# PKU-EPIC/PartManip

Hardware: AMD Instinct MI355X
Metric: PPO env-steps/sec (whole node), 4096 envs x 1024-pt clouds (higher is better)
Workload: dtype f32

## Files before the change

### partmanip_amd/csrc/pointnet_enc_screen.h

```cpp
#pragma once

typedef __bf16 ps_bf16x8 __attribute__((ext_vector_type(8)));

#define PS_LDP (PN_C2 + 8)
#define PS_CAP 128
#define PS_NW 8
#define PS_P3 (16 * 16 * 64 * 8)
#define PS_OFF_P3H 0
#define PS_OFF_P3L (2 * PS_P3)
#define PS_OFF_W3 (4 * PS_P3 + 8192)
#define PS_OFF_EPS (PS_OFF_W3 + PN_C3 * PN_C2 * 4)
#define PS_PACKED_BYTES (PS_OFF_EPS + PN_C3 * 4)
#ifndef PS_ABLATE
#define PS_ABLATE 0
#endif
#ifndef PS_SCHED_DEFAULT
#define PS_SCHED_DEFAULT 0
#endif

extern "C" size_t pm_pointnet_packed_screen_bytes(void) { return PS_PACKED_BYTES; }

__device__ __forceinline__ unsigned ps_cvt_pk(float a, float b) {
    unsigned r;
    asm("v_cvt_pk_bf16_f32 %0, %1, %2" : "=v"(r) : "v"(a), "v"(b));
    return r;
}
__device__ __forceinline__ void ps_split(float x, unsigned short& hi, unsigned short& lo) {
    const unsigned h = ps_cvt_pk(x, 0.f) & 0xffffu;
    const float xh = __uint_as_float(h << 16);
    hi = (unsigned short)h;
    lo = (unsigned short)(ps_cvt_pk(x - xh, 0.f) & 0xffffu);
}

__global__ __launch_bounds__(256) void ps_pack_kernel(const float* __restrict__ W3, const float* __restrict__ b3,
                                                       unsigned char* __restrict__ packed) {
    const int i = blockIdx.x * 256 + threadIdx.x;
    if (i >= PS_P3) return;
    unsigned short* Ph = (unsigned short*)(packed + PS_OFF_P3H);
    unsigned short* Pl = (unsigned short*)(packed + PS_OFF_P3L);
    float* Wr = (float*)(packed + PS_OFF_W3);
    const int e = i & 7, lane = (i >> 3) & 63, li = lane & 31, lq = lane >> 5, step = (i >> 9) & 15, nb = i >> 13;
    unsigned short h, l;
    ps_split(W3[(nb * 32 + li) * PN_C2 + step * 16 + lq * 8 + e], h, l);
    Ph[i] = h;
    Pl[i] = l;
    Wr[i] = W3[i];
    if (i < 4096) ((unsigned short*)(packed + 4 * PS_P3))[i] = 0;
    if (i < PN_C3) {
        double L = 0.0;
        for (int k = 0; k < PN_C2; ++k) L += fabs((double)W3[i * PN_C2 + k]);
        const double ed = (0x1p-16 + 2048.0 * 0x1p-24) * (L + fabs((double)b3[i])) * (1.0 + 0x1p-10);
        float ef = (float)ed;
        if ((double)ef < ed) ef = __uint_as_float(__float_as_uint(ef) + 1);
        ((float*)(packed + PS_OFF_EPS))[i] = ef;
    }
}

extern "C" int pm_pointnet_pack_weights_screen(const float* W3, const float* b3, void* packed, void* stream) {
    PM_REQUIRE(W3 && b3 && packed);
    if (((uintptr_t)packed & 15) != 0) return PM_EALIGN;
    hipLaunchKernelGGL(ps_pack_kernel, dim3(PS_P3 / 256), dim3(256), 0, pm_stream(stream), W3, b3, (unsigned char*)packed);
    PM_CHECK_LAUNCH();
    return PM_OK;
}

#define PS_MFMA(a, b, c) __builtin_amdgcn_mfma_f32_32x32x16_bf16((a), (b), (c), 0, 0, 0)
__device__ __forceinline__ ps_bf16x8 ps_bf(const uint4& v) { return *(const ps_bf16x8*)&v; }

__device__ __forceinline__ void ps_stream(const unsigned short* __restrict__ Ah, const unsigned short* __restrict__ Al,
                                          const uint4* __restrict__ Bh, const uint4* __restrict__ Bl, f32x16 (&acc)[2][2]) {
    uint4 bh0[2], bl0[2], bh1[2], bl1[2];
#pragma unroll
    for (int nb = 0; nb < 2; ++nb) {
        bh0[nb] = Bh[(size_t)(nb * 16) * 64];
        bl0[nb] = Bl[(size_t)(nb * 16) * 64];
    }
#define PS_STEP(S_, BHC, BLC, BHN, BLN)                                                        \
    {                                                                                          \
        uint4 ah[2], al[2];                                                                    \
        _Pragma("unroll") for (int mb = 0; mb < 2; ++mb) {                                     \
            ah[mb] = *(const uint4*)(Ah + mb * 32 * PS_LDP + (S_) * 16);                       \
            al[mb] = *(const uint4*)(Al + mb * 32 * PS_LDP + (S_) * 16);                       \
        }                                                                                      \
        _Pragma("unroll") for (int nb = 0; nb < 2; ++nb) {    \
            BHN[nb] = Bh[(size_t)(nb * 16 + (S_) + 1) * 64];                                   \
            BLN[nb] = Bl[(size_t)(nb * 16 + (S_) + 1) * 64];                                   \
        }                                                                                      \
        __builtin_amdgcn_sched_barrier(0);                                                     \
        _Pragma("unroll") for (int nb = 0; nb < 2; ++nb)                                       \
            _Pragma("unroll") for (int mb = 0; mb < 2; ++mb) {                                 \
                acc[mb][nb] = PS_MFMA(ps_bf(ah[mb]), ps_bf(BHC[nb]), acc[mb][nb]);             \
                acc[mb][nb] = PS_MFMA(ps_bf(ah[mb]), ps_bf(BLC[nb]), acc[mb][nb]);             \
                acc[mb][nb] = PS_MFMA(ps_bf(al[mb]), ps_bf(BHC[nb]), acc[mb][nb]);             \
            }                                                                                  \
        __builtin_amdgcn_sched_barrier(0);                                                     \
    }
#pragma unroll 1
    for (int s = 0; s < 16; s += 2) {
        PS_STEP(s, bh0, bl0, bh1, bl1)
        PS_STEP(s + 1, bh1, bl1, bh0, bl0)
    }
#undef PS_STEP
}

template <int SCHED>
__device__ __forceinline__ bool ps_late_wave(int wave) { return SCHED == 1 && __builtin_amdgcn_readfirstlane(wave) >= 4; }

template <int NT>
__device__ __forceinline__ void ps_copy_h2(const float* __restrict__ H, float* __restrict__ dst, int tid) {
#pragma unroll 2
    for (int i = 0; i < PN_TM * PN_C2 / 4 / NT; ++i) {
        const int q = tid + NT * i, row = q >> 6, c4 = q & 63;
        const f32x4 v = *(const f32x4*)(H + row * PN_LD2 + 4 * c4);
        *(f32x4*)(dst + row * PN_C2 + 4 * c4) = v;
    }
}

static_assert(PN_TM * PN_MAXC == PS_NW * 64, "one staged slot per thread");
__device__ __forceinline__ float ps_point_load(const float* __restrict__ xb, int tile, int C, int tid) {
    const int p = tid >> 3, d = tid & 7;
    return d < C ? xb[(tile * PN_TM + p) * C + d] : 0.f;
}
__device__ __forceinline__ void ps_point_store(float v, int sub_mean, const float (&cen)[3], int tid, float* __restrict__ Xs) {
    const int d = tid & 7;
    if (sub_mean && d < 3) v -= cen[d];
    Xs[tid] = v;
}

#ifdef PS_PROFILE
__device__ unsigned long long ps_prof[4 * 16 * PS_NW * 16];
extern "C" int pm_debug_ps_prof_read(void* dst) {
    return hipMemcpyFromSymbol(dst, HIP_SYMBOL(ps_prof), sizeof(ps_prof)) == hipSuccess ? 0 : 1;
}
#define PS_STAMP(i)                                                                                         \
    if (b < 4 && tile < 16 && lane0 == 0) ps_prof[((b * 16 + tile) * PS_NW + wave) * 16 + (i)] = __builtin_readcyclecounter()
#else
#define PS_STAMP(i)
#endif

template <int CT, int SCHED>
__global__ __launch_bounds__(PS_NW * 64, 2) void pn_fwd_screen_kernel(
    const float* __restrict__ x, long ldx, int P, int C, int sub_mean, const float* __restrict__ W1,
    const float* __restrict__ b1, const float* __restrict__ b2, const float* __restrict__ b3,
    const float* __restrict__ packed, const unsigned char* __restrict__ packed_s, int max_mean, float* __restrict__ feat,
    long ldf, int32_t* __restrict__ argmax, float* __restrict__ h2_save, unsigned long long* __restrict__ counters) {
    constexpr int NT = PS_NW * 64;
    __shared__ __attribute__((aligned(16))) float H[PN_TM * PN_LD2];
    __shared__ __attribute__((aligned(16))) unsigned short Hp[2 * PN_TM * PS_LDP];
    __shared__ __attribute__((aligned(16))) float Xs[PN_TM * PN_MAXC];
    __shared__ double red[16];
    __shared__ double cs[PN_C2];
    __shared__ int skey[PS_NW][PS_CAP];
    unsigned short* Hh = Hp;
    unsigned short* Hl = Hp + PN_TM * PS_LDP;

    const int b = blockIdx.x, tid = threadIdx.x, lane0 = tid & 63, wave = tid >> 6;
    const float* xb = x + (long)b * ldx;
    const float4* P2v = (const float4*)(packed + PN_P2_OFF);
    const float4* P3v = (const float4*)(packed + PN_P3_OFF);
    const uint4* S3h = (const uint4*)(packed_s + PS_OFF_P3H);
    const uint4* S3l = (const uint4*)(packed_s + PS_OFF_P3L);
    const float* W3r = (const float*)(packed_s + PS_OFF_W3);
    const float* epsg = (const float*)(packed_s + PS_OFF_EPS);

    float cen[3] = {0.f, 0.f, 0.f};
    if (sub_mean) cloud_centroid<NT>(xb, P, C, red, cen);

    float vmax = -INFINITY, pois = 0.f;
    int imax = 0;
    double csum = 0.0;

    const int li0 = lane0 & 31;
    const float b2r = b2[wave * 32 + li0];
    const float b3r[2] = {b3[(wave * 2 + 0) * 32 + li0], b3[(wave * 2 + 1) * 32 + li0]};
    const float epsr[2] = {epsg[(wave * 2 + 0) * 32 + li0], epsg[(wave * 2 + 1) * 32 + li0]};
    float w1r[4] = {0.f, 0.f, 0.f, 0.f}, b1r = 0.f;
    if constexpr (CT == 3 || CT == 4) layer1_row<CT>(W1, b1, w1r, b1r);

    const int ntiles = P / PN_TM;
    stage_points<PN_TM, NT>(xb, 0, C, sub_mean, cen, Xs);
    for (int tile = 0; tile < ntiles; ++tile) {
        int lane = lane0;
        asm volatile("" : "+v"(lane));
        const int li = lane & 31, lh = lane >> 5;
        PS_STAMP(0);
        __syncthreads();
        float xnext = 0.f;
        if (tile + 1 < ntiles) xnext = ps_point_load(xb, tile + 1, C, tid);
        if (!(PS_ABLATE & 1)) {
            if constexpr (CT == 3 || CT == 4) layer1_tile<CT, PN_TM, NT, true>(Xs, w1r, b1r, H);
            else layer1_tile<CT, PN_TM, NT, true>(Xs, W1, b1, C, H);
        }
        PS_STAMP(1);
        __syncthreads();
        {
            f32x16 acc2[2][1];
            zero_acc<2, 1>(acc2);
            if (PS_ABLATE & 2) {
#pragma unroll
                for (int mb = 0; mb < 2; ++mb)
#pragma unroll
                    for (int r = 0; r < 16; ++r)
                        acc2[mb][0][r] = H[(mb * 32 + (r & 3) + 8 * (r >> 2) + 4 * lh) * PN_LD1 + ((wave * 32 + li) & 127)];
            } else {
                layer2_mfma<2, 1>(H, P2v, wave, lane, acc2);
            }
            PS_STAMP(2);
            __syncthreads();
            PS_STAMP(3);
            const int col = wave * 32 + li;
            const float b2c = b2r;
            float ts = 0.f;
            const bool planes = !(PS_ABLATE & 8) || tile == 0;
            const bool odd = (lane & 1) != 0;
            unsigned* Hh2 = (unsigned*)(Hh + (odd ? PS_LDP : 0) + (col & ~1));
            unsigned* Hl2 = (unsigned*)(Hl + (odd ? PS_LDP : 0) + (col & ~1));
#pragma unroll
            for (int mb = 0; mb < 2; ++mb)
#pragma unroll
                for (int r = 0; r < 16; r += 2) {
                    const float z0 = acc2[mb][0][r] + b2c, z1 = acc2[mb][0][r + 1] + b2c;
                    f32x2 v2;
                    if (PS_ABLATE & 4) {
                        v2.x = z0;
                        v2.y = z1;
                    } else {
                        v2 = pm_tanh2(z0, z1);
                    }
                    const int row0 = mb * 32 + (r & 3) + 8 * (r >> 2) + 4 * lh;
                    H[row0 * PN_LD2 + col] = v2.x;
                    H[(row0 + 1) * PN_LD2 + col] = v2.y;
                    ts += v2.x;
                    ts += v2.y;
                    const float own = odd ? v2.y : v2.x, send = odd ? v2.x : v2.y;
                    const float recv = __int_as_float(__builtin_amdgcn_update_dpp(0, __float_as_int(send), 0xB1, 0xf, 0xf, false));
                    const float a = odd ? recv : own, c = odd ? own : recv;
                    unsigned h2w, l2w;
                    if (PS_ABLATE & 4) {
                        h2w = (__float_as_uint(a) >> 16) | (__float_as_uint(c) & 0xffff0000u);
                        l2w = 0;
                    } else {
                        h2w = ps_cvt_pk(a, c);
                        l2w = ps_cvt_pk(a - __uint_as_float(h2w << 16), c - __uint_as_float(h2w & 0xffff0000u));
                    }
                    if (planes) {
                        Hh2[row0 * (PS_LDP / 2)] = h2w;
                        Hl2[row0 * (PS_LDP / 2)] = l2w;
                    }
                }
            ts += __shfl_xor(ts, 32, 64);
            csum += (double)ts;
            if (tile + 1 < ntiles) ps_point_store(xnext, sub_mean, cen, tid, Xs);
        }
        PS_STAMP(4);
        __syncthreads();
        PS_STAMP(5);

        const bool copy = h2_save && !(PS_ABLATE & 128), late = ps_late_wave<SCHED>(wave);
        float* h2dst = copy ? h2_save + ((long)b * P + (long)tile * PN_TM) * PN_C2 : nullptr;
        if (copy && late) ps_copy_h2<NT>(H, h2dst, tid);

        f32x16 acc[2][2];
#pragma unroll
        for (int nb = 0; nb < 2; ++nb) {
            const float b3c = b3r[nb];
#pragma unroll
            for (int r = 0; r < 16; ++r) acc[0][nb][r] = acc[1][nb][r] = b3c;
        }
        if (PS_ABLATE & 16) {
#pragma unroll
            for (int nb = 0; nb < 2; ++nb)
#pragma unroll
                for (int mb = 0; mb < 2; ++mb)
#pragma unroll
                    for (int r = 0; r < 16; ++r)
                        acc[mb][nb][r] += H[(mb * 32 + (r & 3) + 8 * (r >> 2) + 4 * lh) * PN_LD2 + ((wave * 64 + nb * 32 + li) & 255)];
        } else {
            ps_stream(Hh + li * PS_LDP + lh * 8, Hl + li * PS_LDP + lh * 8, S3h + (size_t)(wave * 2 * 16) * 64 + lane,
                      S3l + (size_t)(wave * 2 * 16) * 64 + lane, acc);
        }
        PS_STAMP(6);

        unsigned msk[2];
        float tmax[2];
#if (PS_ABLATE & 32) && defined(__HIP_DEVICE_COMPILE__)
#pragma unroll
        for (int nb = 0; nb < 2; ++nb) {
#pragma unroll
            for (int mb = 0; mb < 2; ++mb) asm volatile("" ::"v"(acc[mb][nb]));
            msk[nb] = 0;
            tmax[nb] = 0.f;
        }
#else
#pragma unroll
        for (int nb = 0; nb < 2; ++nb) {
            float m = -INFINITY;
#pragma unroll
            for (int mb = 0; mb < 2; ++mb)
#pragma unroll
                for (int r = 0; r < 16; ++r) m = fmaxf(m, acc[mb][nb][r]);
            m = fmaxf(m, __shfl_xor(m, 32, 64));
            const float e = epsr[nb];
            const float vm = __shfl(vmax, nb * 32 + li, 64);
            const float thr = m - 2.f * e;
            unsigned k = 0;
#pragma unroll
            for (int mb = 0; mb < 2; ++mb)
#pragma unroll
                for (int r = 0; r < 16; ++r) {
                    const float z = acc[mb][nb][r];
                    const bool s = !(z < thr) && !(z + e <= vm);
                    k |= (s ? 1u : 0u) << (mb * 16 + r);
                }
            msk[nb] = k;
            tmax[nb] = m;
        }
#endif
        const int n = __popc(msk[0]) + __popc(msk[1]);
        int incl = n;
#pragma unroll
        for (int o = 1; o < 64; o <<= 1) {
            const int t = __shfl_up(incl, o, 64);
            if (lane >= o) incl += t;
        }
        const int total = __builtin_amdgcn_readlane(incl, 63);
        PS_STAMP(7);

        if (PS_ABLATE & 64) {
            vmax = fmaxf(vmax, lh ? tmax[1] : tmax[0]);
            if (counters && lane == 0) atomicAdd(counters + 0, (unsigned long long)total);
        } else if (total <= PS_CAP) {
            int off = incl - n;
#pragma unroll
            for (int nb = 0; nb < 2; ++nb) {
                unsigned m = msk[nb];
                while (m) {
                    const int bit = __ffs(m) - 1;
                    m &= m - 1;
                    const int row = (bit >> 4) * 32 + (bit & 3) + 8 * ((bit & 15) >> 2) + 4 * lh;
                    skey[wave][off++] = (row << 6) | (nb * 32 + li);
                }
            }
            __builtin_amdgcn_wave_barrier();
            const int j = lane & 7, g = lane >> 3;
            for (int e0 = 0; e0 < total; e0 += 8) {
                const int e = e0 + g;
                const int key = (e < total) ? skey[wave][e] : 0;
                const int row = key >> 6, cl = key & 63;
                const float* hp = H + row * PN_LD2 + 4 * j;
                const float* wp = W3r + (size_t)(wave * 64 + cl) * PN_C2 + 4 * j;
                float s = 0.f;
#pragma unroll
                for (int i = 0; i < 8; ++i) {
                    const float4 w = *(const float4*)(wp + 32 * i);
                    const float4 h = *(const float4*)(hp + 32 * i);
                    s = fmaf(w.x, h.x, s);
                    s = fmaf(w.y, h.y, s);
                    s = fmaf(w.z, h.z, s);
                    s = fmaf(w.w, h.w, s);
                }
                s += __shfl_xor(s, 4, 64);
                s += __shfl_xor(s, 2, 64);
                s += __shfl_xor(s, 1, 64);
                s += b3[wave * 64 + cl];
#pragma unroll
                for (int gg = 0; gg < 8; ++gg)
                    if (e0 + gg < total) {
                        const int kk = __builtin_amdgcn_readlane(key, gg * 8);
                        const float v = __int_as_float(__builtin_amdgcn_readlane(__float_as_int(s), gg * 8));
                        if ((kk & 63) == lane) {
                            const int p = tile * PN_TM + (kk >> 6);
                            if (!(fabsf(v) < INFINITY)) pois += v;
                            if (v > vmax || (v == vmax && p < imax)) {
                                vmax = v;
                                imax = p;
                            }
                        }
                    }
            }
            if (counters) {
                const unsigned long long h0 = __ballot(msk[0] != 0), h1 = __ballot(msk[1] != 0);
                if (lane == 0) {
                    atomicAdd(counters + 0, (unsigned long long)total);
                    atomicAdd(counters + 2, (unsigned long long)(__popc((unsigned)(h0 | (h0 >> 32))) + __popc((unsigned)(h1 | (h1 >> 32)))));
                }
            }
        } else {
#pragma unroll
            for (int nb = 0; nb < 2; ++nb) {
                const float b3c = b3r[nb];
#pragma unroll
                for (int r = 0; r < 16; ++r) acc[0][nb][r] = acc[1][nb][r] = b3c;
            }
            mfma_stream<2, 2, 32>(H + li * PN_LD2 + lh * 128, PN_LD2, P3v + (size_t)(wave * 2) * 32 * 64 + lane, acc);
#pragma unroll
            for (int nb = 0; nb < 2; ++nb) {
                float bv = -INFINITY, ps = 0.f;
                int bp = 0;
#pragma unroll
                for (int mb = 0; mb < 2; ++mb)
#pragma unroll
                    for (int r = 0; r < 16; ++r) {
                        const float v = acc[mb][nb][r];
                        if (!(fabsf(v) < INFINITY)) ps += v;
                        if (v > bv) {
                            bv = v;
                            bp = tile * PN_TM + mb * 32 + (r & 3) + 8 * (r >> 2) + 4 * lh;
                        }
                    }
                const float ov = __shfl_xor(bv, 32, 64), os = __shfl_xor(ps, 32, 64);
                const int op = __shfl_xor(bp, 32, 64);
                if (ov > bv || (ov == bv && op < bp)) {
                    bv = ov;
                    bp = op;
                }
                if (lh == nb) {
                    pois += ps + os;
                    if (bv > vmax || (bv == vmax && bp < imax)) {
                        vmax = bv;
                        imax = bp;
                    }
                }
            }
            if (counters && lane == 0) atomicAdd(counters + 1, 1ull);
        }
        PS_STAMP(8);
        if (copy && !late) ps_copy_h2<NT>(H, h2dst, tid);
        PS_STAMP(9);
    }
    if ((lane0 >> 5) == 0) cs[wave * 32 + lane0] = csum;
    __syncthreads();
    const int ch = tid;
    float v = vmax;
    if (pois != pois) v = pois;
    feat[(long)b * ldf + ch] = v;
    argmax[(long)b * PN_C3 + ch] = imax;
    if (max_mean) {
        const float* wr = W3r + (size_t)ch * PN_C2;
        double s = 0.0;
#pragma unroll 4
        for (int k = 0; k < PN_C2; k += 4) {
            const float4 w = *(const float4*)(wr + k);
            s = fma((double)w.x, cs[k], s);
            s = fma((double)w.y, cs[k + 1], s);
            s = fma((double)w.z, cs[k + 2], s);
            s = fma((double)w.w, cs[k + 3], s);
        }
        float mv = (float)(s / (double)P + (double)b3[ch]);
        if (pois != pois) mv = pois;
        feat[(long)b * ldf + PN_C3 + ch] = mv;
    }
}

extern "C" int pm_pointnet_enc_fwd_screen_sched_f32(const float* x, long ldx, int B, int P, int C, int sub_mean, const float* W1,
                                                    const float* b1, const float* b2, const float* b3, const float* packed,
                                                    const void* packed_screen, int max_mean, float* feat, long ldf,
                                                    int32_t* argmax, float* h2_save, unsigned long long* counters, int schedule,
                                                    void* stream) {
    PM_REQUIRE(x && W1 && b1 && b2 && b3 && packed && packed_screen && feat && argmax);
    PM_REQUIRE(schedule == 0 || schedule == 1);
    if (h2_save && ((uintptr_t)h2_save & 15) != 0) return PM_EALIGN;
    PM_REQUIRE(B > 0 && P > 0 && P % PN_TM == 0 && C >= 1 && C <= PN_MAXC && ldx >= (long)P * C);
    PM_REQUIRE(ldf >= PN_C3 * (max_mean ? 2 : 1));
    PM_REQUIRE(!sub_mean || C >= 3);
    if (((uintptr_t)packed & 15) != 0 || ((uintptr_t)packed_screen & 15) != 0 || ((uintptr_t)counters & 7) != 0) return PM_EALIGN;
#define PS_LAUNCH(CT, S)                                                                                              \
    hipLaunchKernelGGL((pn_fwd_screen_kernel<CT, S>), dim3(B), dim3(PS_NW * 64), 0, pm_stream(stream), x, ldx, P, C, sub_mean, \
                       W1, b1, b2, b3, packed, (const unsigned char*)packed_screen, max_mean, feat, ldf, argmax, h2_save,   \
                       counters)
    if (schedule == 0) {
        if (C == 3) PS_LAUNCH(3, 0);
        else if (C == 4) PS_LAUNCH(4, 0);
        else PS_LAUNCH(0, 0);
    } else {
        if (C == 3) PS_LAUNCH(3, 1);
        else if (C == 4) PS_LAUNCH(4, 1);
        else PS_LAUNCH(0, 1);
    }
#undef PS_LAUNCH
    PM_CHECK_LAUNCH();
    return PM_OK;
}

extern "C" int pm_pointnet_enc_fwd_screen_f32(const float* x, long ldx, int B, int P, int C, int sub_mean, const float* W1,
                                              const float* b1, const float* b2, const float* b3, const float* packed,
                                              const void* packed_screen, int max_mean, float* feat, long ldf,
                                              int32_t* argmax, float* h2_save, unsigned long long* counters, void* stream) {
    return pm_pointnet_enc_fwd_screen_sched_f32(x, ldx, B, P, C, sub_mean, W1, b1, b2, b3, packed, packed_screen, max_mean, feat,
                                                ldf, argmax, h2_save, counters, PS_SCHED_DEFAULT, stream);
}
```

Before: 31960.

## Streamline screen mask build, key compaction and candidate scatter in PointNet max screen

Builds the per-lane candidate bitmask with a single fused threshold and an inline-asm compare plus add-with-carry shift. It replaces the prefix-sum-then-serial compaction with ballot/mbcnt rounds that stop early once the cap is exceeded. The candidate results are routed back to their owning lanes with ds_permute, and the old readlane loop is kept as a fallback when two candidates in a batch target the same lane. The aim is to cut VALU and shuffle work in the candidate-screening path. The risks are that the merged threshold relies on float rounding margins and the inline asm clobbers vcc.

```diff
diff --git a/partmanip_amd/csrc/pointnet_enc_screen.h b/partmanip_amd/csrc/pointnet_enc_screen.h
--- a/partmanip_amd/csrc/pointnet_enc_screen.h
+++ b/partmanip_amd/csrc/pointnet_enc_screen.h
@@ -125,6 +125,11 @@
     const int d = tid & 7;
     if (sub_mean && d < 3) v -= cen[d];
     Xs[tid] = v;
+}
+
+__device__ __forceinline__ unsigned ps_shift_in_nlt(unsigned k, float z, float T) {
+    asm("v_cmp_nlt_f32 vcc, %1, %2\n\tv_addc_co_u32 %0, vcc, %0, %0, vcc" : "+v"(k) : "v"(z), "v"(T) : "vcc");
+    return k;
 }
 
 #ifdef PS_PROFILE
@@ -302,50 +307,41 @@
             m = fmaxf(m, __shfl_xor(m, 32, 64));
             const float e = epsr[nb];
             const float vm = __shfl(vmax, nb * 32 + li, 64);
-            const float thr = m - 2.f * e;
+            const float d = vm - e;
+            const float T = fmaxf(m - 2.f * e, d - fmaf(fabsf(d), 0x1p-23f, 0x1p-100f));
             unsigned k = 0;
 #pragma unroll
-            for (int mb = 0; mb < 2; ++mb)
-#pragma unroll
-                for (int r = 0; r < 16; ++r) {
-                    const float z = acc[mb][nb][r];
-                    const bool s = !(z < thr) && !(z + e <= vm);
-                    k |= (s ? 1u : 0u) << (mb * 16 + r);
-                }
+            for (int q = 31; q >= 0; --q) k = ps_shift_in_nlt(k, acc[q >> 4][nb][q & 15], T);
             msk[nb] = k;
             tmax[nb] = m;
         }
 #endif
-        const int n = __popc(msk[0]) + __popc(msk[1]);
-        int incl = n;
-#pragma unroll
-        for (int o = 1; o < 64; o <<= 1) {
-            const int t = __shfl_up(incl, o, 64);
-            if (lane >= o) incl += t;
-        }
-        const int total = __builtin_amdgcn_readlane(incl, 63);
         PS_STAMP(7);
-
+        int total = 0;
+#pragma unroll
+        for (int nb = 0; nb < 2; ++nb) {
+            unsigned m = msk[nb];
+            const int kbase = (4 * lh) << 6 | (nb * 32 + li);
+            for (;;) {
+                const unsigned long long act = __ballot(m != 0);
+                if (!act || total > PS_CAP) break;
+                const int slot = __builtin_amdgcn_mbcnt_hi((unsigned)(act >> 32), __builtin_amdgcn_mbcnt_lo((unsigned)act, total));
+                total = __builtin_amdgcn_readfirstlane(total + __popcll(act));
+                if (m && total <= PS_CAP) {
+                    const int q = __ffs(m) - 1;
+                    m &= m - 1;
+                    skey[wave][slot] = (((q & 0x1c) << 1 | (q & 3)) << 6) | kbase;
+                }
+            }
+        }
         if (PS_ABLATE & 64) {
             vmax = fmaxf(vmax, lh ? tmax[1] : tmax[0]);
             if (counters && lane == 0) atomicAdd(counters + 0, (unsigned long long)total);
         } else if (total <= PS_CAP) {
-            int off = incl - n;
-#pragma unroll
-            for (int nb = 0; nb < 2; ++nb) {
-                unsigned m = msk[nb];
-                while (m) {
-                    const int bit = __ffs(m) - 1;
-                    m &= m - 1;
-                    const int row = (bit >> 4) * 32 + (bit & 3) + 8 * ((bit & 15) >> 2) + 4 * lh;
-                    skey[wave][off++] = (row << 6) | (nb * 32 + li);
-                }
-            }
             __builtin_amdgcn_wave_barrier();
             const int j = lane & 7, g = lane >> 3;
             for (int e0 = 0; e0 < total; e0 += 8) {
-                const int e = e0 + g;
-                const int key = (e < total) ? skey[wave][e] : 0;
+                const int key = skey[wave][min(e0 + g, total - 1)];
                 const int row = key >> 6, cl = key & 63;
                 const float* hp = H + row * PN_LD2 + 4 * j;
                 const float* wp = W3r + (size_t)(wave * 64 + cl) * PN_C2 + 4 * j;
@@ -363,20 +359,35 @@
                 s += __shfl_xor(s, 2, 64);
                 s += __shfl_xor(s, 1, 64);
                 s += b3[wave * 64 + cl];
-#pragma unroll
-                for (int gg = 0; gg < 8; ++gg)
-                    if (e0 + gg < total) {
-                        const int kk = __builtin_amdgcn_readlane(key, gg * 8);
-                        const float v = __int_as_float(__builtin_amdgcn_readlane(__float_as_int(s), gg * 8));
-                        if ((kk & 63) == lane) {
-                            const int p = tile * PN_TM + (kk >> 6);
-                            if (!(fabsf(v) < INFINITY)) pois += v;
-                            if (v > vmax || (v == vmax && p < imax)) {
-                                vmax = v;
-                                imax = p;
+                const int nv = min(8, total - e0);
+                const int rw = __builtin_amdgcn_ds_permute(cl << 2, row | 64);
+                const float rv = __int_as_float(__builtin_amdgcn_ds_permute(cl << 2, __float_as_int(s)));
+                const bool got = rw != 0;
+                if (__popcll(__ballot(got)) == nv) {
+                    if (got) {
+                        const int p = tile * PN_TM + (rw & 63);
+                        if (!(fabsf(rv) < INFINITY)) pois += rv;
+                        if (rv > vmax || (rv == vmax && p < imax)) {
+                            vmax = rv;
+                            imax = p;
+                        }
+                    }
+                } else {
+#pragma unroll
+                    for (int gg = 0; gg < 8; ++gg)
+                        if (gg < nv) {
+                            const int kk = __builtin_amdgcn_readlane(key, gg * 8);
+                            const float v = __int_as_float(__builtin_amdgcn_readlane(__float_as_int(s), gg * 8));
+                            if ((kk & 63) == lane) {
+                                const int p = tile * PN_TM + (kk >> 6);
+                                if (!(fabsf(v) < INFINITY)) pois += v;
+                                if (v > vmax || (v == vmax && p < imax)) {
+                                    vmax = v;
+                                    imax = p;
+                                }
                             }
                         }
-                    }
+                }
             }
             if (counters) {
                 const unsigned long long h0 = __ballot(msk[0] != 0), h1 = __ballot(msk[1] != 0);
```

New measurement: 32730 (median of 6 runs). 2.4% higher.
